# chernistry/sentio

Hardware: AMD Instinct MI355X
Metric: chat_qps (higher is better)
Workload: dtype bf16; 1 GPU; model=llama3-8b, encoder=sentio-encoder-base, reranker=sentio-reranker-base, global_batch=32, seq_len=2048, docs_per_gpu=10000000, total_docs=10000000, parallelism=dp1+index-shard1, device=cuda

## Files before the change

### sentio_amd/engines/transformer.py

```python

from __future__ import annotations

import math
import os

import torch

from sentio_amd import ops
from sentio_amd.engines.configs import ModelConfig
from sentio_amd.parallel.tp import (TPContext, linear_row_parallel,
                                    shard_columns, shard_qkv, shard_rows)


def _dtype(name: str) -> torch.dtype:
    return {"bf16": torch.bfloat16, "fp16": torch.float16, "fp32": torch.float32}[name]


class TransformerWeights:

    def __init__(self, cfg: ModelConfig, device: str, dtype: torch.dtype,
                 seed: int = 1234, tp: TPContext | None = None):
        self.cfg = cfg
        self.device = device
        self.dtype = dtype
# ... 127 lines not shown
            raise ValueError("kv scales must be finite and positive")
        rows.append(kv)
    for sc, kv in zip(scales, rows):
        kv = kv.to(sc.device)
        sc[:2].copy_(kv)
        sc[2:].copy_(torch.reciprocal(kv))


class Transformer:

    def __init__(self, cfg: ModelConfig, device: str = "cpu",
                 dtype: str | torch.dtype = "bf16", seed: int = 1234,
                 tp: TPContext | None = None):
        self.cfg = cfg
        self.device = device
        self.tp = tp or TPContext()
        if self.tp.enabled:
            assert cfg.n_heads % self.tp.world == 0
            assert cfg.n_kv_heads % self.tp.world == 0
        self.h_local = cfg.n_heads // self.tp.world
        self.hkv_local = cfg.n_kv_heads // self.tp.world
        self.dtype = _dtype(dtype) if isinstance(dtype, str) else dtype
        if device == "cpu":
            self.dtype = torch.float32
        self.w = TransformerWeights(cfg, device, self.dtype, seed, self.tp)
        cos, sin = ops.torch_ref.rope_tables(cfg.max_seq, cfg.head_dim,
                                             cfg.rope_base, device)
        self.rope_cos, self.rope_sin = cos, sin
        self.scale = 1.0 / math.sqrt(cfg.head_dim)
        self.decode_attn = (
            ops.decode_attention_bmm
            if os.environ.get("SENTIO_DECODE_ATTN") == "bmm"
            else ops.decode_attention)

    def _attn(self, x: torch.Tensor, layer: dict, pos: torch.Tensor,
              cache: KVCache | None, layer_idx: int,
              kv_lens: torch.Tensor | None, q_off: int = 0) -> torch.Tensor:
        cfg = self.cfg
        B, S, d = x.shape
        hd = cfg.head_dim
        H, Hkv = self.h_local, self.hkv_local
        qkv = torch.nn.functional.linear(x.view(B * S, d), layer["wqkv"])
        qkv = qkv.view(B, S, -1)
        q_end = H * hd
        k_end = q_end + Hkv * hd
        q = qkv[..., :q_end].reshape(B, S, H, hd)
        k = qkv[..., q_end:k_end].reshape(B, S, Hkv, hd)
        v = qkv[..., k_end:].reshape(B, S, Hkv, hd)
        q = ops.rope_apply(q, self.rope_cos, self.rope_sin, pos)
        k = ops.rope_apply(k, self.rope_cos, self.rope_sin, pos)

        if cache is not None and cache.fp8:
            raise ValueError("prefill writes exact K/V: run it into a bf16 "
                             "staging KVCache and splice with "
                             "ops.kv_store_fp8")
        if cache is not None:
            kc, vc = cache.k[layer_idx], cache.v[layer_idx]
            idx = pos.long()
            bidx = torch.arange(B, device=x.device).unsqueeze(1).expand(B, S)
            kc[bidx.reshape(-1), :, idx.reshape(-1)] = \
                k.reshape(B * S, Hkv, hd).to(kc.dtype)
            vc[bidx.reshape(-1), :, idx.reshape(-1)] = \
                v.reshape(B * S, Hkv, hd).to(vc.dtype)

        if S == 1 and cache is not None:
            seq_lens = (pos[:, 0] + 1).to(torch.int32)
# ... 28 lines not shown
            gu = torch.nn.functional.linear(xx, layer["w_gate_up"])
            y = ops.swiglu_packed(gu)
            out = linear_row_parallel(y, layer["w_down"], self.tp)
        return out.view(B, S, d)

    def forward_hidden(
        self, tokens: torch.Tensor, pos: torch.Tensor | None = None,
        cache: KVCache | None = None, kv_lens: torch.Tensor | None = None,
        q_off: int = 0,
    ) -> torch.Tensor:
        B, S = tokens.shape
        if pos is None:
            pos = torch.arange(S, device=tokens.device).unsqueeze(0).expand(B, S)
        x = self.w.tok_emb[tokens.reshape(-1)].view(B, S, self.cfg.dim)
        eps = self.cfg.norm_eps
        layers = self.w.layers
        n = len(layers)
        normed = ops.rmsnorm(x, layers[0]["attn_norm"], eps)
        for i, layer in enumerate(layers):
            a = self._attn(normed, layer, pos, cache, i, kv_lens, q_off=q_off)
            normed, x = ops.rmsnorm_residual(a, x, layer["ffn_norm"], eps)
            f = self._ffn(normed, layer)
            w_next = layers[i + 1]["attn_norm"] if i + 1 < n else self.w.final_norm
            normed, x = ops.rmsnorm_residual(f, x, w_next, eps)
        return normed

    def _decode_fused(self, x: torch.Tensor) -> bool:
        return self.decode_attn is ops.decode_attention and x.is_cuda

    def _attn_decode(self, normed: torch.Tensor, layer: dict, cache: KVCache,
                     layer_idx: int,
                     attn_lens: torch.Tensor | None) -> torch.Tensor:
        B = normed.shape[0]
        d = self.cfg.dim
        hd = self.cfg.head_dim
        qkv = ops.lt_linear(normed.view(B, d), layer["wqkv"])
        if cache.fp8:
            sc = cache.scales[layer_idx]
            out = ops.decode_attention_fused_fp8(
                qkv, cache.k[layer_idx], cache.v[layer_idx], self.rope_cos,
                self.rope_sin, cache.seq_lens, sc[0], sc[1], sc[2], sc[3],
                self.scale)
        elif self._decode_fused(qkv):
            out = ops.decode_attention_fused(
                qkv, cache.k[layer_idx], cache.v[layer_idx], self.rope_cos,
                self.rope_sin, cache.seq_lens, self.scale)
        else:
            q = ops.decode_qkv_prep(qkv, cache.k[layer_idx],
                                    cache.v[layer_idx], self.rope_cos,
                                    self.rope_sin, cache.seq_lens)
            out = self.decode_attn(q, cache.k[layer_idx], cache.v[layer_idx],
                                   attn_lens, self.scale)
        out = linear_row_parallel(out.view(B, self.h_local * hd),
                                  layer["wo"], self.tp, linear=ops.lt_linear)
        return out.view(B, 1, d)

    def forward_decode(self, tokens: torch.Tensor, cache: KVCache) -> torch.Tensor:
        B = tokens.shape[0]
        x = self.w.tok_emb[tokens.reshape(-1)].view(B, 1, self.cfg.dim)
        eps = self.cfg.norm_eps
        layers = self.w.layers
        n = len(layers)
        attn_lens = (None if self._decode_fused(x) else cache.seq_lens + 1)
        normed = ops.rmsnorm(x, layers[0]["attn_norm"], eps)
        for i, layer in enumerate(layers):
            a = self._attn_decode(normed, layer, cache, i, attn_lens)
            normed, x = ops.rmsnorm_residual(a, x, layer["ffn_norm"], eps)
            f = self._ffn(normed, layer)
            w_next = layers[i + 1]["attn_norm"] if i + 1 < n else self.w.final_norm
            normed, x = ops.rmsnorm_residual(f, x, w_next, eps)
        return normed

    def logits(self, hidden: torch.Tensor,
               last_idx: torch.Tensor | None = None) -> torch.Tensor:
        B, S, d = hidden.shape
        if last_idx is None:
            last = hidden[:, -1, :]
        else:
            last = hidden[torch.arange(B, device=hidden.device),
                          last_idx.to(hidden.device).long()]
        if B <= 64 and self.device != "cpu":
            return ops.lt_linear(last.contiguous(), self.w.lm_head).float()
        return torch.nn.functional.linear(last, self.w.lm_head).float()

    def prefill(self, tokens: torch.Tensor, cache: KVCache,
                lens: torch.Tensor | None = None) -> torch.Tensor:
        B, S = tokens.shape
        lens_i = None if lens is None else lens.to(torch.int32)
        hidden = self.forward_hidden(tokens, cache=cache, kv_lens=lens_i)
        if lens_i is None:
            cache.seq_lens[:] = S
            last_idx = None
        else:
            cache.seq_lens.copy_(lens_i)
            last_idx = lens_i.long() - 1
        return self.logits(hidden, last_idx)

    def prefill_suffix(self, suffix_tokens: torch.Tensor, cache: KVCache,
                       prefix_len: int,
                       suffix_lens: torch.Tensor | None = None) -> torch.Tensor:
        B, S = suffix_tokens.shape
        pos = (prefix_len + torch.arange(S, device=suffix_tokens.device)
               ).unsqueeze(0).expand(B, S)
# ... 17 lines not shown
```

### sentio_amd/ops/__init__.py

```python

from __future__ import annotations

import math

import torch

from sentio_amd.ops import torch_ref

_hip = None
_hip_err: str | None = None


def _load_hip():
    global _hip, _hip_err
    if _hip is not None or _hip_err is not None:
        return _hip
    try:
        from sentio_amd.ops import _sentio_hip

        _hip = _sentio_hip
    except ImportError as e:
        _hip_err = str(e)
    return _hip


def hip_available() -> bool:
    return _load_hip() is not None


def _require_hip():
    m = _load_hip()
    if m is None:
        raise RuntimeError(
            "sentio_amd HIP extension (_sentio_hip) is not built but a CUDA "
            "tensor reached an op. Build it with `python setup.py "
            f"build_ext --inplace` (PYTORCH_ROCM_ARCH=gfx950). Import error: {_hip_err}"
        )
    return m


def _on_gpu(*tensors: torch.Tensor) -> bool:
    return any(t.is_cuda for t in tensors if isinstance(t, torch.Tensor))



def rmsnorm(x, weight, eps: float = 1e-5):
    if _on_gpu(x):
        return _require_hip().rmsnorm(x.contiguous(), weight.contiguous(), eps)
    return torch_ref.rmsnorm(x, weight, eps)


def rmsnorm_residual(x, residual, weight, eps: float = 1e-5):
    if _on_gpu(x):
        return _require_hip().rmsnorm_residual(
            x.contiguous(), residual.contiguous(), weight.contiguous(), eps
        )
    return torch_ref.rmsnorm_residual(x, residual, weight, eps)


def rope_apply(x, cos, sin, pos):
    if _on_gpu(x):
        return _require_hip().rope_apply(
            x.contiguous(), cos.contiguous(), sin.contiguous(), pos.contiguous()
        )
    return torch_ref.rope_apply(x, cos, sin, pos)


def decode_qkv_prep(qkv, k_cache, v_cache, cos, sin, seq_lens):
    if _on_gpu(qkv):
        return _require_hip().decode_qkv_prep(
            qkv.contiguous(), k_cache, v_cache, cos, sin, seq_lens)
    return torch_ref.decode_qkv_prep(qkv, k_cache, v_cache, cos, sin, seq_lens)


def swiglu(gate, up):
    if _on_gpu(gate):
        return _require_hip().swiglu(gate.contiguous(), up.contiguous())
    return torch_ref.swiglu(gate, up)


def swiglu_packed(gu):
    if _on_gpu(gu):
        return _require_hip().swiglu_packed(gu.contiguous())
    return torch_ref.swiglu_packed(gu)


def softmax(x, dim: int = -1):
    if _on_gpu(x):
        if dim not in (-1, x.ndim - 1):
            x = x.transpose(dim, -1).contiguous()
# ... 310 lines not shown
    _check_slot_array(seed, "seed", S, torch.int64, dev)
    _check_slot_array(step, "step", S, torch.int32, dev)
    if active is not None:
        _check_slot_array(active, "active", S, torch.uint8, dev)
    if slot is None:
        if R != S:
            raise ValueError(f"without a slot table logits must have one row "
                             f"per slot: {R} rows for {S} slots")
    elif isinstance(slot, torch.Tensor):
        _check_slot_array(slot, "slot", R, torch.int32, dev)
    else:
        slot = [int(s) for s in slot]
        if len(slot) != R:
            raise ValueError(f"{len(slot)} slots for {R} logits rows")
        if any(s < 0 or s >= S for s in slot):
            raise ValueError(f"slots {slot} outside [0, {S})")
        if len(set(slot)) != len(slot):
            raise ValueError(f"duplicate slots in {slot}")
        slot = torch.tensor(slot, dtype=torch.int32, device=dev)
    if _on_gpu(logits):
        _require_hip().sample_slots(logits.contiguous(), slot, temperature,
                                    top_k, top_p, seed, step, active, tok)
        return
    torch_ref.sample_slots(logits, slot, temperature, top_k, top_p, seed,
                           step, active, tok)


def skinny_gemm(x, w):
    if _on_gpu(x):
        return _require_hip().skinny_gemm(x.contiguous(), w.contiguous())
    return torch.nn.functional.linear(x.float(), w.float()).to(x.dtype)


_lt_ok = True


def lt_linear(x, w):
    global _lt_ok
    import os

    if (_lt_ok and _on_gpu(x)
            and os.environ.get("SENTIO_LT_GEMM", "1") != "0"):
        try:
            return _require_hip().lt_gemm_tn(x.contiguous(), w.contiguous())
        except RuntimeError as exc:
            if "rc=5" not in str(exc):
                _lt_ok = False
    return torch.nn.functional.linear(x, w)


def gemm_bf16(a, b):
    if _on_gpu(a):
        return _require_hip().gemm_bf16(a.contiguous(), b.contiguous())
    return (a.float() @ b.float()).to(a.dtype)


__all__ = [
    "rmsnorm", "rmsnorm_residual", "rope_apply", "decode_qkv_prep", "decode_attention_fused", "decode_attention_fused_fp8", "kv_store_fp8", "swiglu", "swiglu_packed", "softmax",
    "attention", "attention_cache", "decode_attention", "decode_attention_bmm", "mean_pool_l2norm", "cosine_topk",
    "bm25_score", "cosine_scores", "fuse_topk", "lt_linear", "sample_token", "sample_filtered", "sample_slots", "sample_support", "gemm_bf16", "skinny_gemm", "hip_available", "torch_ref",
]
```

### sentio_amd/ops/csrc/bindings.hip

```cpp
#include <torch/extension.h>
#include <c10/hip/HIPStream.h>
#include <hip/hip_runtime.h>
#include <cstdlib>
#include <tuple>

#include "sentio_kernels.h"

namespace {

void check_hip(hipError_t e, const char* what) {
  TORCH_CHECK(e == hipSuccess, "sentio HIP kernel '", what,
              "' failed: ", hipGetErrorString(e));
}

hipStream_t stream() {
  return c10::hip::getCurrentHIPStream().stream();
}

void check_bf16_cuda(const torch::Tensor& t, const char* name) {
  TORCH_CHECK(t.is_cuda(), name, " must be on GPU");
  TORCH_CHECK(t.scalar_type() == torch::kBFloat16, name, " must be bf16");
  TORCH_CHECK(t.is_contiguous(), name, " must be contiguous");
}

torch::Tensor rmsnorm(torch::Tensor x, torch::Tensor w, double eps) {
  check_bf16_cuda(x, "x");
  check_bf16_cuda(w, "w");
  const int D = x.size(-1);
  const long rows = x.numel() / D;
  auto y = torch::empty_like(x);
  check_hip(sentio_rmsnorm(x.data_ptr(), w.data_ptr(), y.data_ptr(), rows, D,
                           (float)eps, stream()), "rmsnorm");
  return y;
}

std::vector<torch::Tensor> rmsnorm_residual(torch::Tensor x, torch::Tensor res,
// ... 418 lines not shown
}

void kv_store_fp8(torch::Tensor src_k, torch::Tensor src_v, torch::Tensor kc,
                  torch::Tensor vc, torch::Tensor rows, long S,
                  torch::Tensor k_inv, torch::Tensor v_inv) {
  check_bf16_cuda(src_k, "src_k");
  check_bf16_cuda(src_v, "src_v");
  TORCH_CHECK(src_k.dim() == 4 && src_v.sizes() == src_k.sizes(),
              "sources must be two [n,Hkv,S_src,D] tensors of equal shape");
  check_caches_u8(kc, vc);
  const long n = src_k.size(0), Hkv = kc.size(1), Smax = kc.size(2);
  const long D = kc.size(3), S_src = src_k.size(2);
  TORCH_CHECK(src_k.size(1) == Hkv && src_k.size(3) == D,
              "source and cache kv heads / head dim differ");
  TORCH_CHECK(D % 8 == 0, "head dim must be a multiple of 8, got ", D);
  TORCH_CHECK(S >= 0 && S <= S_src && S <= Smax,
              "S must be <= min(S_src, Smax), got ", S);
  TORCH_CHECK(rows.is_cuda() && rows.device() == kc.device() &&
              rows.scalar_type() == torch::kInt && rows.is_contiguous() &&
              rows.dim() == 1 && rows.numel() == n,
              "rows must be a contiguous i32 [n] tensor on the caches' device");
  TORCH_CHECK(src_k.device() == kc.device(), "sources and caches on "
              "different devices");
  check_kv_scale(k_inv, kc, Hkv, "k_inv");
  check_kv_scale(v_inv, kc, Hkv, "v_inv");
  check_hip(sentio_kv_store_fp8(
                src_k.data_ptr(), src_v.data_ptr(), kc.data_ptr(),
                vc.data_ptr(), rows.data_ptr<int>(), k_inv.data_ptr<float>(),
                v_inv.data_ptr<float>(), (int)n, (int)kc.size(0), (int)Hkv,
                (int)S_src, (int)S, (int)Smax, (int)D, stream()),
            "kv_store_fp8");
}

torch::Tensor gemm_bf16(torch::Tensor a, torch::Tensor b) {
  check_bf16_cuda(a, "a");
  check_bf16_cuda(b, "b");
  const int M = a.size(0), K = a.size(1), N = b.size(1);
  TORCH_CHECK(b.size(0) == K, "inner dims mismatch");
  auto c = torch::empty({M, N}, a.options());
  check_hip(sentio_gemm_bf16(a.data_ptr(), b.data_ptr(), c.data_ptr(), M, N, K,
                             stream()), "gemm_bf16");
  return c;
}

}

torch::Tensor skinny_gemm(torch::Tensor x, torch::Tensor w) {
  check_bf16_cuda(x, "x");
  check_bf16_cuda(w, "w");
  TORCH_CHECK(x.dim() == 2 && w.dim() == 2, "x [M,K], w [N,K]");
  TORCH_CHECK(x.size(1) == w.size(1), "K mismatch");
  const int M = x.size(0), K = x.size(1), N = w.size(0);
  auto out = torch::empty({M, N}, x.options());
  check_hip(sentio_skinny_gemm(x.data_ptr(), w.data_ptr(), out.data_ptr(),
                               M, K, N, stream()), "skinny_gemm");
  return out;
}

std::vector<torch::Tensor> fuse_topk(torch::Tensor d_ids, torch::Tensor d_scores,
                                     torch::Tensor s_ids, torch::Tensor s_scores,
                                     int64_t top_k, int64_t method,
                                     double rrf_k, double dw, double sw) {
  TORCH_CHECK(d_ids.is_cuda() && d_ids.scalar_type() == torch::kLong, "d_ids i64 GPU");
  TORCH_CHECK(s_ids.scalar_type() == torch::kLong, "s_ids i64");
  const int B = d_ids.size(0), Kd = d_ids.size(1), Ks = s_ids.size(1);
  auto out_ids = torch::empty({B, top_k}, d_ids.options());
// ... 33 lines not shown
  const int B = q.size(0), S = q.size(1), H = q.size(2), D = q.size(3);
  const int Hkv = kc.size(1), Smax = kc.size(2);
  auto out = torch::empty_like(q);
  check_hip(sentio_flash_attn_cache(q.data_ptr(), kc.data_ptr(), vc.data_ptr(),
                                    out.data_ptr(),
                                    kv_lens.contiguous().data_ptr<int>(), B, S,
                                    H, Hkv, Smax, D, (float)scale, (int)q_off,
                                    stream()), "flash_attn_cache");
  return out;
}

PYBIND11_MODULE(TORCH_EXTENSION_NAME, m) {
  m.def("rmsnorm", &rmsnorm);
  m.def("rmsnorm_residual", &rmsnorm_residual);
  m.def("swiglu", &swiglu);
  m.def("swiglu_packed", &swiglu_packed);
  m.def("rope_apply", &rope_apply);
  m.def("decode_qkv_prep", &decode_qkv_prep);
  m.def("softmax_lastdim", &softmax_lastdim);
  m.def("mean_pool_l2norm", &mean_pool_l2norm);
  m.def("sample_token", &sample_token);
  m.def("sample_support", &sample_support);
  m.def("sample_filtered", &sample_filtered);
  m.def("sample_slots", &sample_slots);
  m.def("cosine_scores", &cosine_scores);
  m.def("bm25_score", &bm25_score);
  m.def("flash_attn", &flash_attn);
  m.def("flash_attn_cache", &flash_attn_cache);
  m.def("decode_attn", &decode_attn);
  m.def("decode_attn_fused", &decode_attn_fused);
  m.def("decode_attn_fused_fp8", &decode_attn_fused_fp8);
  m.def("kv_store_fp8", &kv_store_fp8);
  m.def("decode_attn_plan", &decode_attn_plan);
  m.def("gemm_bf16", &gemm_bf16);
  m.def("skinny_gemm", &skinny_gemm);
  m.def("fuse_topk", &fuse_topk);
  m.def("lt_gemm_tn", &lt_gemm_tn);
}
```

### sentio_amd/ops/csrc/elementwise.hip

```cpp
#include "common.h"
#include "sentio_kernels.h"

template <int VEC>
__global__ void rmsnorm_kernel(const bf16* __restrict__ x,
                               const bf16* __restrict__ w,
                               bf16* __restrict__ y, int D, float eps) {
  __shared__ float scratch[32];
  const long row = blockIdx.x;
  const bf16* xr = x + row * (long)D;
  bf16* yr = y + row * (long)D;

  float ss = 0.f;
  for (int d = threadIdx.x * VEC; d < D; d += blockDim.x * VEC) {
    if (VEC == 8) {
      bf16x8 v = *reinterpret_cast<const bf16x8*>(xr + d);
#pragma unroll
      for (int j = 0; j < 8; ++j) { float f = bits2f(v[j]); ss += f * f; }
    } else {
      float f = bf2f(xr[d]);
      ss += f * f;
    }
  }
  ss = block_sum(ss, scratch);
  const float inv = rsqrtf(ss / (float)D + eps);
// ... 27 lines not shown
  bf16* yr = y + row * (long)D;
  bf16* hr = h + row * (long)D;

  float ss = 0.f;
  for (int d = threadIdx.x * VEC; d < D; d += blockDim.x * VEC) {
    if (VEC == 8) {
      bf16x8 a = *reinterpret_cast<const bf16x8*>(xr + d);
      bf16x8 b = *reinterpret_cast<const bf16x8*>(rr + d);
      bf16x8 o;
#pragma unroll
      for (int j = 0; j < 8; ++j) {
        float f = bits2f(a[j]) + bits2f(b[j]);
        o[j] = f2bits(f);
        ss += f * f;
      }
      *reinterpret_cast<bf16x8*>(hr + d) = o;
    } else {
      float f = bf2f(xr[d]) + bf2f(rr[d]);
      hr[d] = f2bf(f);
      ss += f * f;
    }
  }
  ss = block_sum(ss, scratch);
  const float inv = rsqrtf(ss / (float)D + eps);
  for (int d = threadIdx.x * VEC; d < D; d += blockDim.x * VEC) {
    if (VEC == 8) {
      bf16x8 v = *reinterpret_cast<const bf16x8*>(hr + d);
      bf16x8 wv = *reinterpret_cast<const bf16x8*>(w + d);
      bf16x8 o;
#pragma unroll
      for (int j = 0; j < 8; ++j)
        o[j] = f2bits(bits2f(v[j]) * inv * bits2f(wv[j]));
      *reinterpret_cast<bf16x8*>(yr + d) = o;
    } else {
      yr[d] = f2bf(bf2f(hr[d]) * inv * bf2f(w[d]));
    }
  }
}

__global__ void swiglu_kernel(const bf16* __restrict__ gate,
                              const bf16* __restrict__ up,
                              bf16* __restrict__ out, long n8) {
  for (long i = blockIdx.x * (long)blockDim.x + threadIdx.x; i < n8;
       i += (long)gridDim.x * blockDim.x) {
    bf16x8 g = reinterpret_cast<const bf16x8*>(gate)[i];
    bf16x8 u = reinterpret_cast<const bf16x8*>(up)[i];
    bf16x8 o;
#pragma unroll
    for (int j = 0; j < 8; ++j) {
      float gf = bits2f(g[j]);
      float s = gf / (1.f + __expf(-gf));
      o[j] = f2bits(s * bits2f(u[j]));
    }
    reinterpret_cast<bf16x8*>(out)[i] = o;
  }
}
__global__ void swiglu_packed_kernel(const bf16* __restrict__ gu,
                                     bf16* __restrict__ out, long rows, int F) {
  const int f8 = F / 8;
  for (long i = blockIdx.x * (long)blockDim.x + threadIdx.x;
       i < rows * (long)f8; i += (long)gridDim.x * blockDim.x) {
    const long r = i / f8;
    const int c8 = (int)(i % f8);
    const bf16* row = gu + r * (long)(2 * F);
    bf16x8 g = *reinterpret_cast<const bf16x8*>(row + c8 * 8);
    bf16x8 u = *reinterpret_cast<const bf16x8*>(row + F + c8 * 8);
// ... 183 lines not shown
}

extern "C" {

hipError_t sentio_rmsnorm(const void* x, const void* w, void* y, long rows,
                          int D, float eps, hipStream_t stream) {
  dim3 block(256);
  if (D % 8 == 0)
    hipLaunchKernelGGL((rmsnorm_kernel<8>), dim3((unsigned)rows), block, 0,
                       stream, (const bf16*)x, (const bf16*)w, (bf16*)y, D, eps);
  else
    hipLaunchKernelGGL((rmsnorm_kernel<1>), dim3((unsigned)rows), block, 0,
                       stream, (const bf16*)x, (const bf16*)w, (bf16*)y, D, eps);
  HIP_CHECK_LAUNCH();
  return hipSuccess;
}

hipError_t sentio_rmsnorm_residual(const void* x, const void* res, const void* w,
                                   void* y, void* h, long rows, int D,
                                   float eps, hipStream_t stream) {
  dim3 block(256);
  if (D % 8 == 0)
    hipLaunchKernelGGL((rmsnorm_residual_kernel<8>), dim3((unsigned)rows), block,
                       0, stream, (const bf16*)x, (const bf16*)res,
                       (const bf16*)w, (bf16*)y, (bf16*)h, D, eps);
  else
    hipLaunchKernelGGL((rmsnorm_residual_kernel<1>), dim3((unsigned)rows), block,
                       0, stream, (const bf16*)x, (const bf16*)res,
                       (const bf16*)w, (bf16*)y, (bf16*)h, D, eps);
  HIP_CHECK_LAUNCH();
  return hipSuccess;
}

hipError_t sentio_swiglu(const void* gate, const void* up, void* out, long n,
                         hipStream_t stream) {
  long n8 = n / 8;
  if (n8 > 0) {
    long blocks = (n8 + 255) / 256;
    if (blocks > 2048) blocks = 2048;
    hipLaunchKernelGGL(swiglu_kernel, dim3((unsigned)blocks), dim3(256), 0,
                       stream, (const bf16*)gate, (const bf16*)up, (bf16*)out, n8);
  }
  long tail = n - n8 * 8;
  if (tail > 0) {
    hipLaunchKernelGGL(swiglu_tail_kernel, dim3(1), dim3(256), 0, stream,
                       (const bf16*)gate, (const bf16*)up, (bf16*)out,
                       n8 * 8, n);
  }
  HIP_CHECK_LAUNCH();
  return hipSuccess;
}

hipError_t sentio_rope(const void* x, void* y, const float* cosT,
                       const float* sinT, const int* pos, int B, int S, int H,
                       int D, hipStream_t stream) {
  long total = (long)B * S * H * (D / 2);
  long blocks = (total + 255) / 256;
  if (blocks > 2048) blocks = 2048;
  hipLaunchKernelGGL(rope_kernel, dim3((unsigned)blocks), dim3(256), 0, stream,
                     (const bf16*)x, (bf16*)y, cosT, sinT, pos, S, H, D, total);
  HIP_CHECK_LAUNCH();
  return hipSuccess;
}

hipError_t sentio_swiglu_packed(const void* gu, void* out, long rows, int F,
                                hipStream_t stream) {
// ... 56 lines not shown
```

### sentio_amd/ops/csrc/gemm.hip

```cpp
#include "common.h"
#include "sentio_kernels.h"

typedef __bf16 bf16x8_t __attribute__((ext_vector_type(8)));
typedef float f32x4_t __attribute__((ext_vector_type(4)));

#define BM 128
#define BN 128
#define BK 64
#define BT_STRIDE (BK * 2 + 16)

__device__ __forceinline__ void stage_tile_glds(
    const bf16* __restrict__ gsrc, int ld, int rows, int row0, int col0,
    char* lds_dst, int tid) {
  const int total_chunks = rows * BK / 8;
  for (int c = tid; c < total_chunks; c += 256) {
    const int elem = c * 8;
    const int r = elem / BK;
    const int col = elem % BK;
    auto gp = (const __attribute__((address_space(1))) unsigned int*)
        (gsrc + (long)(row0 + r) * ld + col0 + col);
    auto lp = (__attribute__((address_space(3))) unsigned int*)
        (lds_dst + (long)elem * 2);
    __builtin_amdgcn_global_load_lds(gp, lp, 16, 0, 0);
  }
// ... 156 lines not shown
#pragma unroll
    for (int u = 0; u < UNR; ++u) {
      acc[0] = __builtin_amdgcn_mfma_f32_16x16x32_bf16(a[u], b0[u], acc[0],
                                                       0, 0, 0);
      if (MTILES > 1)
        acc[1] = __builtin_amdgcn_mfma_f32_16x16x32_bf16(a[u], b1[u], acc[1],
                                                         0, 0, 0);
    }
  }
  for (; k0 < K; k0 += 32) {
    bf16x8_t a = *reinterpret_cast<const bf16x8_t*>(wrow + k0 + kofs);
    bf16x8_t b0 = *reinterpret_cast<const bf16x8_t*>(xrow0 + k0 + kofs);
    if (!m_ok0) { bf16x8_t z = {}; b0 = z; }
    acc[0] = __builtin_amdgcn_mfma_f32_16x16x32_bf16(a, b0, acc[0], 0, 0, 0);
    if (MTILES > 1) {
      bf16x8_t b1 = *reinterpret_cast<const bf16x8_t*>(xrow1 + k0 + kofs);
      if (!m_ok1) { bf16x8_t z = {}; b1 = z; }
      acc[1] = __builtin_amdgcn_mfma_f32_16x16x32_bf16(a, b1, acc[1], 0, 0, 0);
    }
  }

#pragma unroll
  for (int mt = 0; mt < MTILES; ++mt) {
    const int m = mt * 16 + arow;
    if (m >= M) continue;
#pragma unroll
    for (int r = 0; r < 4; ++r) {
      const int n = n0 + (lane >> 4) * 4 + r;
      if (n < N) out[(long)m * N + n] = f2bf(acc[mt][r]);
    }
  }
}

extern "C" {

hipError_t sentio_skinny_gemm(const void* x, const void* w, void* out, int M,
                              int K, int N, hipStream_t stream) {
  if (M > 32 || (K % 32)) return hipErrorInvalidValue;
  dim3 grid((N + 63) / 64);
  if (M <= 16)
    hipLaunchKernelGGL((skinny_gemm_kernel<16>), grid, dim3(256), 0, stream,
                       (const bf16*)x, (const bf16*)w, (bf16*)out, M, K, N);
  else
    hipLaunchKernelGGL((skinny_gemm_kernel<32>), grid, dim3(256), 0, stream,
                       (const bf16*)x, (const bf16*)w, (bf16*)out, M, K, N);
  HIP_CHECK_LAUNCH();
  return hipSuccess;
}

hipError_t sentio_gemm_bf16(const void* A, const void* B, void* C, int M,
                            int N, int K, hipStream_t stream) {
  if (M % BM || N % BN || K % BK) return hipErrorInvalidValue;
  const int nwg = (M / BM) * (N / BN);
  size_t lds = 2 * (BM * BK * 2 + BN * BT_STRIDE);
  hipLaunchKernelGGL(gemm_bf16_kernel, dim3(nwg), dim3(256), lds, stream,
                     (const bf16*)A, (const bf16*)B, (bf16*)C, M, N, K);
  HIP_CHECK_LAUNCH();
  return hipSuccess;
}

}
```

### sentio_amd/ops/csrc/sentio_kernels.h

```cpp
#pragma once

#include <hip/hip_runtime.h>

extern "C" {

hipError_t sentio_rmsnorm(const void* x, const void* w, void* y, long rows,
                          int D, float eps, hipStream_t stream);
hipError_t sentio_rmsnorm_residual(const void* x, const void* res,
                                   const void* w, void* y, void* h, long rows,
                                   int D, float eps, hipStream_t stream);
hipError_t sentio_swiglu(const void* gate, const void* up, void* out, long n,
                         hipStream_t stream);
hipError_t sentio_swiglu_packed(const void* gu, void* out, long rows, int F,
                                hipStream_t stream);
hipError_t sentio_rope(const void* x, void* y, const float* cosT,
                       const float* sinT, const int* pos, int B, int S, int H,
                       int D, hipStream_t stream);
hipError_t sentio_decode_qkv_prep(const void* qkv, void* q_out, void* kc,
                                  void* vc, const float* cosT,
                                  const float* sinT, const int* seq_lens,
                                  int B, int H, int Hkv, int D, int Smax,
                                  hipStream_t stream);
hipError_t sentio_softmax(const void* x, void* y, long rows, int D,
                          hipStream_t stream);
hipError_t sentio_mean_pool_l2norm(const void* hidden,
                                   const unsigned char* mask, float* out,
                                   int B, int S, int D, hipStream_t stream);
hipError_t sentio_sample(const float* logits, long* out, float* ws_val,
                         int* ws_idx, int B, int V, float temperature,
                         unsigned seed, hipStream_t stream);

hipError_t sentio_sample_support(const float* logits, const float* temperature,
                                 const int* top_k, const float* top_p,
                                 float* tau, int* count, long B, int V,
                                 hipStream_t stream);
hipError_t sentio_sample_filtered(const float* logits, const float* temperature,
                                  const int* top_k, const float* top_p,
                                  const long* seed, const int* step, long* out,
                                  long B, int V, hipStream_t stream);
hipError_t sentio_sample_slots(const float* logits, const int* slot,
                               const float* temperature, const int* top_k,
                               const float* top_p, const long* seed, int* step,
                               const unsigned char* active, long* tok, long R,
// ... 24 lines not shown
hipError_t sentio_flash_attn_cache(const void* q, const void* kc,
                                   const void* vc, void* out,
                                   const int* kv_lens, int B, int S, int H,
                                   int Hkv, int Smax, int D, float scale,
                                   int q_off, hipStream_t stream);
hipError_t sentio_decode_attn(const void* q, const void* kc, const void* vc,
                              void* out, const int* seq_lens, float* ws_o,
                              float* ws_ml, int splits, int waves, int B,
                              int H, int Hkv, int Smax, int D, float scale,
                              hipStream_t stream);
hipError_t sentio_decode_attn_fused(const void* qkv, void* kc, void* vc,
                                    void* out, const float* cosT,
                                    const float* sinT, const int* seq_lens,
                                    float* ws_o, float* ws_ml, int splits,
                                    int waves, int B, int H, int Hkv,
                                    int Smax, int D, float scale,
                                    hipStream_t stream);
hipError_t sentio_decode_attn_fused_fp8(
    const void* qkv, void* kc, void* vc, void* out, const float* cosT,
    const float* sinT, const int* seq_lens, const float* k_scale,
    const float* v_scale, const float* k_inv, const float* v_inv, float* ws_o,
    float* ws_ml, int splits, int waves, int B, int H, int Hkv, int Smax,
    int D, float scale, hipStream_t stream);
hipError_t sentio_kv_store_fp8(const void* src_k, const void* src_v,
                               void* dst_k, void* dst_v, const int* rows,
                               const float* k_inv, const float* v_inv, int n,
                               int B, int Hkv, int S_src, int S, int Smax,
                               int D, hipStream_t stream);

hipError_t sentio_gemm_bf16(const void* A, const void* B, void* C, int M,
                            int N, int K, hipStream_t stream);
hipError_t sentio_skinny_gemm(const void* x, const void* w, void* out, int M,
                              int K, int N, hipStream_t stream);
int sentio_lt_gemm_tn(const void* x, const void* w, void* out, int M, int N,
                      int K, hipStream_t stream);

}
```

### sentio_amd/ops/torch_ref.py

```python

from __future__ import annotations

import math

import torch


def rmsnorm(x: torch.Tensor, weight: torch.Tensor, eps: float = 1e-5) -> torch.Tensor:
    xf = x.float()
    rms = xf.pow(2).mean(dim=-1, keepdim=True).add(eps).rsqrt()
    return (xf * rms * weight.float()).to(x.dtype)


def rmsnorm_residual(
    x: torch.Tensor, residual: torch.Tensor, weight: torch.Tensor, eps: float = 1e-5
) -> tuple[torch.Tensor, torch.Tensor]:
    h = (x.float() + residual.float())
    rms = h.pow(2).mean(dim=-1, keepdim=True).add(eps).rsqrt()
    y = (h * rms * weight.float()).to(x.dtype)
    return y, h.to(x.dtype)


def rope_tables(
    max_seq: int, head_dim: int, base: float = 500000.0, device: str = "cpu"
) -> tuple[torch.Tensor, torch.Tensor]:
    inv = 1.0 / (
        base ** (torch.arange(0, head_dim, 2, device=device).float() / head_dim)
    )
    t = torch.arange(max_seq, device=device).float()
    freqs = torch.outer(t, inv)
    return freqs.cos(), freqs.sin()


def rope_apply(
    x: torch.Tensor, cos: torch.Tensor, sin: torch.Tensor, pos: torch.Tensor
) -> torch.Tensor:
    B, S, H, D = x.shape
    c = cos[pos.long()].unsqueeze(2)
    s = sin[pos.long()].unsqueeze(2)
    xf = x.float().view(B, S, H, D // 2, 2)
    x0, x1 = xf[..., 0], xf[..., 1]
    out = torch.stack((x0 * c - x1 * s, x0 * s + x1 * c), dim=-1)
    return out.view(B, S, H, D).to(x.dtype)


def swiglu(gate: torch.Tensor, up: torch.Tensor) -> torch.Tensor:
    return (torch.nn.functional.silu(gate.float()) * up.float()).to(gate.dtype)


def softmax(x: torch.Tensor, dim: int = -1) -> torch.Tensor:
    return torch.softmax(x.float(), dim=dim).to(x.dtype)


# ... 299 lines not shown
```

Baseline: 19.99 requests/s.

## Add split-K MFMA decode GEMM for wo/down with partial-sum fused rmsnorm

Adds a custom split-K bf16 MFMA kernel for the skinny decode GEMMs (wo and w_down, M<=32). It writes f32 partial slabs, and the following rmsnorm_residual kernel reduces the partials while it adds the residual. The goal is more parallel blocks over K for small-batch decode than the library GEMM gives, so more of the weight-streaming bandwidth gets used. In exchange it adds f32 partial traffic and a heuristic split plan, selected automatically when there is no TP and the dtype is bf16 on GPU.

```diff
diff --git a/sentio_amd/engines/transformer.py b/sentio_amd/engines/transformer.py
--- a/sentio_amd/engines/transformer.py
+++ b/sentio_amd/engines/transformer.py
@@ -183,6 +183,19 @@
             ops.decode_attention_bmm
             if os.environ.get("SENTIO_DECODE_ATTN") == "bmm"
             else ops.decode_attention)
+        self.splitk_wo, self.splitk_down = self._plan_decode_gemm()
+
+    def _plan_decode_gemm(self) -> tuple[bool, bool]:
+        mode = os.environ.get("SENTIO_DECODE_GEMM", "auto")
+        if (mode == "lt" or self.tp.enabled or not ops.hip_available()
+                or not str(self.device).startswith("cuda")
+                or self.dtype != torch.bfloat16):
+            return False, False
+        cfg = self.cfg
+        wo = ops.decode_gemm_plan(32, cfg.dim,
+                                  self.h_local * cfg.head_dim)[0] > 0
+        down = ops.decode_gemm_plan(32, cfg.dim, cfg.ffn_dim)[0] > 0
+        return wo and mode != "down", down and mode != "wo"
 
     def _attn(self, x: torch.Tensor, layer: dict, pos: torch.Tensor,
               cache: KVCache | None, layer_idx: int,
@@ -277,6 +290,16 @@
                      layer_idx: int,
                      attn_lens: torch.Tensor | None) -> torch.Tensor:
         B = normed.shape[0]
+        out = self._attn_decode_heads(normed, layer, cache, layer_idx,
+                                      attn_lens)
+        out = linear_row_parallel(out, layer["wo"], self.tp,
+                                  linear=ops.lt_linear)
+        return out.view(B, 1, self.cfg.dim)
+
+    def _attn_decode_heads(self, normed: torch.Tensor, layer: dict,
+                           cache: KVCache, layer_idx: int,
+                           attn_lens: torch.Tensor | None) -> torch.Tensor:
+        B = normed.shape[0]
         d = self.cfg.dim
         hd = self.cfg.head_dim
         qkv = ops.lt_linear(normed.view(B, d), layer["wqkv"])
@@ -296,9 +319,7 @@
                                     self.rope_sin, cache.seq_lens)
             out = self.decode_attn(q, cache.k[layer_idx], cache.v[layer_idx],
                                    attn_lens, self.scale)
-        out = linear_row_parallel(out.view(B, self.h_local * hd),
-                                  layer["wo"], self.tp, linear=ops.lt_linear)
-        return out.view(B, 1, d)
+        return out.view(B, self.h_local * hd)
 
     def forward_decode(self, tokens: torch.Tensor, cache: KVCache) -> torch.Tensor:
         B = tokens.shape[0]
@@ -308,12 +329,27 @@
         n = len(layers)
         attn_lens = (None if self._decode_fused(x) else cache.seq_lens + 1)
         normed = ops.rmsnorm(x, layers[0]["attn_norm"], eps)
+        sk_wo = self.splitk_wo and B <= 32
+        sk_down = self.splitk_down and B <= 32
         for i, layer in enumerate(layers):
-            a = self._attn_decode(normed, layer, cache, i, attn_lens)
-            normed, x = ops.rmsnorm_residual(a, x, layer["ffn_norm"], eps)
-            f = self._ffn(normed, layer)
+            if sk_wo:
+                a = ops.linear_splitk(
+                    self._attn_decode_heads(normed, layer, cache, i,
+                                            attn_lens), layer["wo"])
+                normed, x = ops.rmsnorm_residual_partials(
+                    a, x, layer["ffn_norm"], eps)
+            else:
+                a = self._attn_decode(normed, layer, cache, i, attn_lens)
+                normed, x = ops.rmsnorm_residual(a, x, layer["ffn_norm"], eps)
             w_next = layers[i + 1]["attn_norm"] if i + 1 < n else self.w.final_norm
-            normed, x = ops.rmsnorm_residual(f, x, w_next, eps)
+            if sk_down:
+                gu = ops.lt_linear(normed.view(B, self.cfg.dim),
+                                   layer["w_gate_up"])
+                f = ops.linear_splitk(ops.swiglu_packed(gu), layer["w_down"])
+                normed, x = ops.rmsnorm_residual_partials(f, x, w_next, eps)
+            else:
+                f = self._ffn(normed, layer)
+                normed, x = ops.rmsnorm_residual(f, x, w_next, eps)
         return normed
 
     def logits(self, hidden: torch.Tensor,
diff --git a/sentio_amd/ops/__init__.py b/sentio_amd/ops/__init__.py
--- a/sentio_amd/ops/__init__.py
+++ b/sentio_amd/ops/__init__.py
@@ -56,6 +56,14 @@
             x.contiguous(), residual.contiguous(), weight.contiguous(), eps
         )
     return torch_ref.rmsnorm_residual(x, residual, weight, eps)
+
+
+def rmsnorm_residual_partials(part, residual, weight, eps: float = 1e-5):
+    if _on_gpu(part):
+        y, h = _require_hip().rmsnorm_residual_partials(
+            part.contiguous(), residual.contiguous(), weight.contiguous(), eps)
+        return y, h
+    return torch_ref.rmsnorm_residual_partials(part, residual, weight, eps)
 
 
 def rope_apply(x, cos, sin, pos):
@@ -432,6 +440,21 @@
     return torch.nn.functional.linear(x.float(), w.float()).to(x.dtype)
 
 
+def decode_gemm_plan(M: int, N: int, K: int) -> tuple[int, int, int]:
+    return tuple(_require_hip().decode_gemm_plan(int(M), int(N), int(K)))
+
+
+def linear_splitk(x, w, *, nan_fill: bool = False):
+    if not _on_gpu(x):
+        return torch_ref.linear_splitk(x, w)
+    hip = _require_hip()
+    M, K = x.shape
+    if hip.decode_gemm_plan(M, w.shape[0], K)[0] > 0:
+        return hip.decode_gemm_splitk(x.contiguous(), w.contiguous(),
+                                      bool(nan_fill))
+    return lt_linear(x, w).float().unsqueeze(0)
+
+
 _lt_ok = True
 
 
@@ -458,5 +481,5 @@
 __all__ = [
     "rmsnorm", "rmsnorm_residual", "rope_apply", "decode_qkv_prep", "decode_attention_fused", "decode_attention_fused_fp8", "kv_store_fp8", "swiglu", "swiglu_packed", "softmax",
     "attention", "attention_cache", "decode_attention", "decode_attention_bmm", "mean_pool_l2norm", "cosine_topk",
-    "bm25_score", "cosine_scores", "fuse_topk", "lt_linear", "sample_token", "sample_filtered", "sample_slots", "sample_support", "gemm_bf16", "skinny_gemm", "hip_available", "torch_ref",
+    "bm25_score", "cosine_scores", "fuse_topk", "lt_linear", "linear_splitk", "decode_gemm_plan", "rmsnorm_residual_partials", "sample_token", "sample_filtered", "sample_slots", "sample_support", "gemm_bf16", "skinny_gemm", "hip_available", "torch_ref",
 ]
diff --git a/sentio_amd/ops/csrc/bindings.hip b/sentio_amd/ops/csrc/bindings.hip
--- a/sentio_amd/ops/csrc/bindings.hip
+++ b/sentio_amd/ops/csrc/bindings.hip
@@ -2,6 +2,7 @@
 #include <c10/hip/HIPStream.h>
 #include <hip/hip_runtime.h>
 #include <cstdlib>
+#include <limits>
 #include <tuple>
 
 #include "sentio_kernels.h"
@@ -486,6 +487,78 @@
             "kv_store_fp8");
 }
 
+std::tuple<int, long, long> decode_gemm_plan(long M, long N, long K) {
+  TORCH_CHECK(M > 0 && N > 0 && K > 0, "decode_gemm_plan: empty shape");
+  if (M > 32 || N % 64 || K % 32) return {0, 0, 0};
+  const long tiles = N / 64;
+  auto slab_bytes = [&](long s) { return s * M * N * 4; };
+  if (const char* ov = std::getenv("SENTIO_GEMM_SPLITK")) {
+    const long s = atol(ov);
+    TORCH_CHECK(s >= 1 && s <= 65535 && K % (32 * s) == 0,
+                "SENTIO_GEMM_SPLITK='", ov, "' does not split K=", K,
+                " into slices that are multiples of 32");
+    return {(int)s, tiles * s, slab_bytes(s)};
+  }
+  long best = 0, best_pen = 0, best_depth = 0;
+  for (long s = 1; s <= K / 32; ++s) {
+    if (K % (32 * s) || slab_bytes(s) > (8L << 20)) continue;
+    const long blocks = tiles * s, slice = K / s;
+    if (blocks < 128) continue;
+    const long pen = blocks < 256 ? 256 - blocks
+                   : blocks > 512 ? blocks - 512 : 0;
+    const long depth = slice % 512 == 0 ? 2 : slice % 256 == 0 ? 1 : 0;
+    if (!best || pen < best_pen || (pen == best_pen && depth > best_depth)) {
+      best = s; best_pen = pen; best_depth = depth;
+    }
+  }
+  if (!best) return {0, 0, 0};
+  return {(int)best, tiles * best, slab_bytes(best)};
+}
+
+torch::Tensor decode_gemm_splitk(torch::Tensor x, torch::Tensor w,
+                                 bool nan_fill) {
+  check_bf16_cuda(x, "x");
+  check_bf16_cuda(w, "w");
+  TORCH_CHECK(x.dim() == 2 && w.dim() == 2 && x.size(1) == w.size(1),
+              "x [M,K], w [N,K]");
+  const long M = x.size(0), K = x.size(1), N = w.size(0);
+  const int S = std::get<0>(decode_gemm_plan(M, N, K));
+  TORCH_CHECK(S > 0, "decode_gemm_splitk: no plan for M=", M, " N=", N,
+              " K=", K, " (use the library GEMM)");
+  auto opts = x.options().dtype(torch::kFloat);
+  auto part = nan_fill
+      ? torch::full({S, M, N}, std::numeric_limits<float>::quiet_NaN(), opts)
+      : torch::empty({S, M, N}, opts);
+  check_hip(sentio_decode_gemm_splitk(x.data_ptr(), w.data_ptr(),
+                                      part.data_ptr<float>(), (int)M, (int)K,
+                                      (int)N, S, stream()),
+            "decode_gemm_splitk");
+  return part;
+}
+
+std::vector<torch::Tensor> rmsnorm_residual_partials(torch::Tensor part,
+                                                     torch::Tensor res,
+                                                     torch::Tensor w,
+                                                     double eps) {
+  TORCH_CHECK(part.is_cuda() && part.scalar_type() == torch::kFloat &&
+              part.is_contiguous() && part.dim() >= 2,
+              "part must be a contiguous f32 [S, ..., D] GPU tensor");
+  check_bf16_cuda(res, "res");
+  check_bf16_cuda(w, "w");
+  const int S = part.size(0);
+  const int D = part.size(-1);
+  TORCH_CHECK(S >= 1 && res.numel() * S == part.numel() && res.size(-1) == D &&
+              w.numel() == D, "part [S, rows, D], res [rows, D], w [D]");
+  const long rows = res.numel() / D;
+  auto y = torch::empty_like(res);
+  auto h = torch::empty_like(res);
+  check_hip(sentio_rmsnorm_residual_partials(
+                part.data_ptr<float>(), res.data_ptr(), w.data_ptr(),
+                y.data_ptr(), h.data_ptr(), S, rows, D, (float)eps, stream()),
+            "rmsnorm_residual_partials");
+  return {y, h};
+}
+
 torch::Tensor gemm_bf16(torch::Tensor a, torch::Tensor b) {
   check_bf16_cuda(a, "a");
   check_bf16_cuda(b, "b");
@@ -585,6 +658,9 @@
   m.def("decode_attn_fused_fp8", &decode_attn_fused_fp8);
   m.def("kv_store_fp8", &kv_store_fp8);
   m.def("decode_attn_plan", &decode_attn_plan);
+  m.def("decode_gemm_plan", &decode_gemm_plan);
+  m.def("decode_gemm_splitk", &decode_gemm_splitk);
+  m.def("rmsnorm_residual_partials", &rmsnorm_residual_partials);
   m.def("gemm_bf16", &gemm_bf16);
   m.def("skinny_gemm", &skinny_gemm);
   m.def("fuse_topk", &fuse_topk);
diff --git a/sentio_amd/ops/csrc/elementwise.hip b/sentio_amd/ops/csrc/elementwise.hip
--- a/sentio_amd/ops/csrc/elementwise.hip
+++ b/sentio_amd/ops/csrc/elementwise.hip
@@ -83,6 +83,60 @@
       for (int j = 0; j < 8; ++j)
         o[j] = f2bits(bits2f(v[j]) * inv * bits2f(wv[j]));
       *reinterpret_cast<bf16x8*>(yr + d) = o;
+    } else {
+      yr[d] = f2bf(bf2f(hr[d]) * inv * bf2f(w[d]));
+    }
+  }
+}
+
+template <int VEC>
+__global__ void rmsnorm_residual_partials_kernel(
+    const float* __restrict__ part, const bf16* __restrict__ res,
+    const bf16* __restrict__ w, bf16* __restrict__ y, bf16* __restrict__ h,
+    int S, long rows, int D, float eps) {
+  __shared__ float scratch[32];
+  const long row = blockIdx.x;
+  const long slab = rows * (long)D;
+  const float* pr = part + row * (long)D;
+  const bf16* rr = res + row * (long)D;
+  bf16* yr = y + row * (long)D;
+  bf16* hr = h + row * (long)D;
+
+  float ss = 0.f;
+  for (int d = threadIdx.x * VEC; d < D; d += blockDim.x * VEC) {
+    if (VEC == 4) {
+      f32x4 a = *reinterpret_cast<const f32x4*>(pr + d);
+#pragma unroll 4
+      for (int s = 1; s < S; ++s)
+        a += *reinterpret_cast<const f32x4*>(pr + s * slab + d);
+      bf16x4 b = *reinterpret_cast<const bf16x4*>(rr + d);
+      bf16x4 o;
+#pragma unroll
+      for (int j = 0; j < 4; ++j) {
+        const float f = a[j] + bits2f(b[j]);
+        o[j] = f2bits(f);
+        ss += f * f;
+      }
+      *reinterpret_cast<bf16x4*>(hr + d) = o;
+    } else {
+      float a = pr[d];
+      for (int s = 1; s < S; ++s) a += pr[s * slab + d];
+      const float f = a + bf2f(rr[d]);
+      hr[d] = f2bf(f);
+      ss += f * f;
+    }
+  }
+  ss = block_sum(ss, scratch);
+  const float inv = rsqrtf(ss / (float)D + eps);
+  for (int d = threadIdx.x * VEC; d < D; d += blockDim.x * VEC) {
+    if (VEC == 4) {
+      bf16x4 v = *reinterpret_cast<const bf16x4*>(hr + d);
+      bf16x4 wv = *reinterpret_cast<const bf16x4*>(w + d);
+      bf16x4 o;
+#pragma unroll
+      for (int j = 0; j < 4; ++j)
+        o[j] = f2bits(bits2f(v[j]) * inv * bits2f(wv[j]));
+      *reinterpret_cast<bf16x4*>(yr + d) = o;
     } else {
       yr[d] = f2bf(bf2f(hr[d]) * inv * bf2f(w[d]));
     }
@@ -332,6 +386,28 @@
   return hipSuccess;
 }
 
+hipError_t sentio_rmsnorm_residual_partials(const float* part, const void* res,
+                                            const void* w, void* y, void* h,
+                                            int S, long rows, int D, float eps,
+                                            hipStream_t stream) {
+  if (S < 1 || rows < 1 || D < 1) return hipErrorInvalidValue;
+  const int vec = (D % 4 == 0) ? 4 : 1;
+  int threads = ((D / vec + WAVE - 1) / WAVE) * WAVE;
+  threads = threads > 1024 ? 1024 : threads;
+  if (vec == 4)
+    hipLaunchKernelGGL((rmsnorm_residual_partials_kernel<4>),
+                       dim3((unsigned)rows), dim3(threads), 0, stream, part,
+                       (const bf16*)res, (const bf16*)w, (bf16*)y, (bf16*)h, S,
+                       rows, D, eps);
+  else
+    hipLaunchKernelGGL((rmsnorm_residual_partials_kernel<1>),
+                       dim3((unsigned)rows), dim3(threads), 0, stream, part,
+                       (const bf16*)res, (const bf16*)w, (bf16*)y, (bf16*)h, S,
+                       rows, D, eps);
+  HIP_CHECK_LAUNCH();
+  return hipSuccess;
+}
+
 hipError_t sentio_swiglu(const void* gate, const void* up, void* out, long n,
                          hipStream_t stream) {
   long n8 = n / 8;
diff --git a/sentio_amd/ops/csrc/gemm.hip b/sentio_amd/ops/csrc/gemm.hip
--- a/sentio_amd/ops/csrc/gemm.hip
+++ b/sentio_amd/ops/csrc/gemm.hip
@@ -212,7 +212,171 @@
   }
 }
 
+#define SK_BN 64
+#define SK_THREADS 512
+
+template <int MT, int UNR>
+__launch_bounds__(SK_THREADS, 2)
+__global__ void decode_gemm_splitk_kernel(const bf16* __restrict__ x,
+                                          const bf16* __restrict__ w,
+                                          float* __restrict__ part,
+                                          int M, int K, int N, int kslice) {
+  constexpr int MTILES = MT / 16;
+  constexpr int CK = 2 * UNR * 32;
+  constexpr int PPR = CK / 8;
+  constexpr int NX = MT * PPR / SK_THREADS;
+  constexpr int RPI = SK_THREADS / PPR;
+  static_assert(NX >= 1 && MT * PPR % SK_THREADS == 0, "staging shape");
+  static_assert(MT * CK * 2 >= MT * SK_BN * 4, "epilogue tile fits");
+  __shared__ __attribute__((aligned(16))) char smem[MT * CK * 2];
+
+  const int tid = threadIdx.x;
+  const int lane = tid & (WAVE - 1);
+  const int wid = tid / WAVE;
+  const int strip = wid & 3;
+  const int kg = wid >> 2;
+  const int arow = lane & 15;
+  const int q = lane >> 4;
+  const int tile = blockIdx.x;
+  const int slice = blockIdx.y;
+  const int k_begin = slice * kslice;
+  const int k_end = k_begin + kslice;
+
+  const short* xs_base = reinterpret_cast<const short*>(x);
+  const short* wrow = reinterpret_cast<const short*>(w) +
+      (long)(tile * SK_BN + strip * 16 + arow) * K + q * 8;
+
+  f32x4_t acc[MTILES];
+#pragma unroll
+  for (int mt = 0; mt < MTILES; ++mt) acc[mt] = f32x4_t{};
+
+  const int xt = tid / PPR;
+  const int xp = tid % PPR;
+  const int rd_base[2] = {
+      arow * (CK * 2) + (((kg * 8 + q) ^ arow) * 16),
+      arow * (CK * 2) + (((4 + kg * 8 + q) ^ arow) * 16)};
+
+  struct Chunk { bf16x8 x[NX]; bool ok[NX]; bf16x8 w[UNR]; };
+  auto load_chunk = [&](int c, Chunk& d) {
+    const int kc0 = k_begin + c * CK;
+#pragma unroll
+    for (int i = 0; i < NX; ++i) {
+      const int m = i * RPI + xt;
+      const int k = kc0 + xp * 8;
+      d.ok[i] = m < M && k < k_end;
+      d.x[i] = *reinterpret_cast<const bf16x8*>(
+          xs_base + (long)(d.ok[i] ? m : 0) * K + (d.ok[i] ? k : k_begin));
+    }
+#pragma unroll
+    for (int u = 0; u < UNR; ++u) {
+      const int k = kc0 + ((u & 1) + 2 * kg + 4 * (u >> 1)) * 32;
+      d.w[u] = *reinterpret_cast<const bf16x8*>(wrow + min(k, k_end - 32));
+    }
+    __builtin_amdgcn_sched_barrier(0);
+  };
+  auto stage_x = [&](const Chunk& d) {
+    __syncthreads();
+#pragma unroll
+    for (int i = 0; i < NX; ++i) {
+      bf16x8 v = d.x[i];
+      if (!d.ok[i]) v = bf16x8{};
+      const int piece = (xp ^ xt) ^ ((i * RPI) & 15);
+      *reinterpret_cast<bf16x8*>(smem + (i * RPI + xt) * (CK * 2) +
+                                 piece * 16) = v;
+    }
+    __syncthreads();
+  };
+  auto mma_chunk = [&](const Chunk& d) {
+#pragma unroll
+    for (int u = 0; u < UNR; ++u) {
+      const bf16x8_t a = __builtin_bit_cast(bf16x8_t, d.w[u]);
+#pragma unroll
+      for (int mt = 0; mt < MTILES; ++mt) {
+        const bf16x8_t b = *reinterpret_cast<const bf16x8_t*>(
+            smem + rd_base[u & 1] + (u >> 1) * 256 + mt * 16 * (CK * 2));
+        acc[mt] = __builtin_amdgcn_mfma_f32_16x16x32_bf16(a, b, acc[mt],
+                                                          0, 0, 0);
+      }
+    }
+  };
+
+  const int nchunks = (kslice + CK - 1) / CK;
+  Chunk A, B;
+  int c = 0;
+  load_chunk(0, A);
+  for (; c + 2 < nchunks; c += 2) {
+    stage_x(A);
+    load_chunk(c + 1, B);
+    mma_chunk(A);
+    stage_x(B);
+    load_chunk(c + 2, A);
+    mma_chunk(B);
+  }
+  stage_x(A);
+  if (c + 1 < nchunks) {
+    load_chunk(c + 1, B);
+    mma_chunk(A);
+    stage_x(B);
+    mma_chunk(B);
+  } else {
+    mma_chunk(A);
+  }
+
+  __syncthreads();
+  float* red = reinterpret_cast<float*>(smem);
+  if (kg == 1) {
+#pragma unroll
+    for (int mt = 0; mt < MTILES; ++mt)
+      *reinterpret_cast<f32x4_t*>(red + (mt * 16 + arow) * SK_BN +
+                                  strip * 16 + q * 4) = acc[mt];
+  }
+  __syncthreads();
+  if (kg == 0) {
+#pragma unroll
+    for (int mt = 0; mt < MTILES; ++mt) {
+      f32x4_t* p = reinterpret_cast<f32x4_t*>(red + (mt * 16 + arow) * SK_BN +
+                                              strip * 16 + q * 4);
+      *p = acc[mt] + *p;
+    }
+  }
+  __syncthreads();
+  if (tid < MT * (SK_BN / 4)) {
+    const int row = tid / (SK_BN / 4);
+    const int c4 = tid % (SK_BN / 4);
+    if (row < M)
+      *reinterpret_cast<f32x4_t*>(part + ((long)slice * M + row) * N +
+                                  tile * SK_BN + c4 * 4) =
+          *reinterpret_cast<const f32x4_t*>(red + row * SK_BN + c4 * 4);
+  }
+}
+
+template <int MT, int UNR>
+static void launch_splitk(const void* x, const void* w, float* part, int M,
+                          int K, int N, int S, hipStream_t stream) {
+  hipLaunchKernelGGL((decode_gemm_splitk_kernel<MT, UNR>),
+                     dim3(N / SK_BN, S), dim3(SK_THREADS), 0, stream,
+                     (const bf16*)x, (const bf16*)w, part, M, K, N, K / S);
+}
+
 extern "C" {
+
+hipError_t sentio_decode_gemm_splitk(const void* x, const void* w, float* part,
+                                     int M, int K, int N, int S,
+                                     hipStream_t stream) {
+  if (M < 1 || M > 32 || S < 1 || S > 65535 || K < 32 || N < SK_BN ||
+      (N % SK_BN) || (K % (32 * S)))
+    return hipErrorInvalidValue;
+  const bool deep = (K / S) % 512 == 0;
+  if (M <= 16) {
+    if (deep) launch_splitk<16, 8>(x, w, part, M, K, N, S, stream);
+    else launch_splitk<16, 4>(x, w, part, M, K, N, S, stream);
+  } else {
+    if (deep) launch_splitk<32, 8>(x, w, part, M, K, N, S, stream);
+    else launch_splitk<32, 4>(x, w, part, M, K, N, S, stream);
+  }
+  HIP_CHECK_LAUNCH();
+  return hipSuccess;
+}
 
 hipError_t sentio_skinny_gemm(const void* x, const void* w, void* out, int M,
                               int K, int N, hipStream_t stream) {
diff --git a/sentio_amd/ops/csrc/sentio_kernels.h b/sentio_amd/ops/csrc/sentio_kernels.h
--- a/sentio_amd/ops/csrc/sentio_kernels.h
+++ b/sentio_amd/ops/csrc/sentio_kernels.h
@@ -9,6 +9,10 @@
 hipError_t sentio_rmsnorm_residual(const void* x, const void* res,
                                    const void* w, void* y, void* h, long rows,
                                    int D, float eps, hipStream_t stream);
+hipError_t sentio_rmsnorm_residual_partials(const float* part, const void* res,
+                                            const void* w, void* y, void* h,
+                                            int S, long rows, int D, float eps,
+                                            hipStream_t stream);
 hipError_t sentio_swiglu(const void* gate, const void* up, void* out, long n,
                          hipStream_t stream);
 hipError_t sentio_swiglu_packed(const void* gu, void* out, long rows, int F,
@@ -99,6 +103,9 @@
                             int N, int K, hipStream_t stream);
 hipError_t sentio_skinny_gemm(const void* x, const void* w, void* out, int M,
                               int K, int N, hipStream_t stream);
+hipError_t sentio_decode_gemm_splitk(const void* x, const void* w, float* part,
+                                     int M, int K, int N, int S,
+                                     hipStream_t stream);
 int sentio_lt_gemm_tn(const void* x, const void* w, void* out, int M, int N,
                       int K, hipStream_t stream);
 
diff --git a/sentio_amd/ops/torch_ref.py b/sentio_amd/ops/torch_ref.py
--- a/sentio_amd/ops/torch_ref.py
+++ b/sentio_amd/ops/torch_ref.py
@@ -19,6 +19,20 @@
     rms = h.pow(2).mean(dim=-1, keepdim=True).add(eps).rsqrt()
     y = (h * rms * weight.float()).to(x.dtype)
     return y, h.to(x.dtype)
+
+
+def linear_splitk(x: torch.Tensor, w: torch.Tensor) -> torch.Tensor:
+    return torch.nn.functional.linear(x.float(), w.float()).unsqueeze(0)
+
+
+def rmsnorm_residual_partials(
+    part: torch.Tensor, residual: torch.Tensor, weight: torch.Tensor,
+    eps: float = 1e-5
+) -> tuple[torch.Tensor, torch.Tensor]:
+    h = part.float().sum(dim=0).reshape(residual.shape) + residual.float()
+    rms = h.pow(2).mean(dim=-1, keepdim=True).add(eps).rsqrt()
+    y = (h * rms * weight.float()).to(residual.dtype)
+    return y, h.to(residual.dtype)
 
 
 def rope_tables(
```

Measured after the change: 20.69 requests/s, median of 6. 1.04x the previous value.
